# CVMI-Lab/HybridNeuralRendering

Measured on NVIDIA B200. Metric: train rays/s (fwd+bwd), higher is better.
Workload: dtype f32

## Files before the change

### hybridneuralrendering_b200/csrc/aggregate.cu

```cuda
#include "common.cuh"

#include "hnr.h"
#include "img_common.cuh"

namespace {

constexpr int F_EMB = 32;
constexpr int NF_FEAT = 3;
constexpr int NF_DIST = 5;
constexpr int NF_VIEW = 4;
constexpr int X0_W = F_EMB + 2 * NF_FEAT * F_EMB + 2 * NF_DIST * 6;
constexpr int E_W = 7;
constexpr int HID = 256;
constexpr int X5_W = HID + 2 * NF_VIEW * 3;
constexpr int AUX_C = 45;

__device__ __forceinline__ void rot3(const float* m, float x, float y, float z, float& ox, float& oy, float& oz) {
    ox = x * m[0] + y * m[3] + z * m[6];
    oy = x * m[1] + y * m[4] + z * m[7];
    oz = x * m[2] + y * m[5] + z * m[8];
}

__device__ __forceinline__ bool slot_masked(const int32_t* pidx, const uint8_t* mask, int64_t i) {
    return mask ? (mask[i] == 0) : (pidx[i] < 0);
}

__global__ void nbr_weights_kernel(const float* __restrict__ xyz, const float* __restrict__ conf, const int32_t* __restrict__ pidx,
                                   const uint8_t* __restrict__ mask, const float* __restrict__ loc_w, int64_t S, int K,
                                   float* __restrict__ weight, float* __restrict__ confc, uint8_t* __restrict__ valid) {
    int64_t s = (int64_t)blockIdx.x * blockDim.x + threadIdx.x;
    if (s >= S) return;
    const float lx = loc_w[s * 3], ly = loc_w[s * 3 + 1], lz = loc_w[s * 3 + 2];
    float sum = 0.f;
    bool any = false;
    for (int k = 0; k < K; ++k) {
        int64_t i = s * K + k;
        bool m = slot_masked(pidx, mask, i);
        int64_t g = max(pidx[i], 0);
        float dx = xyz[g * 3] - lx, dy = xyz[g * 3 + 1] - ly, dz = xyz[g * 3 + 2] - lz;
        float u = m ? 0.f : 1.f / fmaxf(sqrtf(dx * dx + dy * dy + dz * dz), 1e-6f);
        weight[i] = u;
        sum += u;
        any |= !m;
        if (confc) confc[i] = conf ? fminf(fmaxf(conf[g], 1e-4f), 1.f) : 1.f;
    }
    float inv = 1.f / fmaxf(sum, 1e-8f);
    for (int k = 0; k < K; ++k) weight[s * K + k] *= inv;
    if (valid) valid[s] = any ? 1 : 0;
}

__global__ void __launch_bounds__(256)
nbr_features_kernel(const float* __restrict__ xyz, const float* __restrict__ xyz_pers, const float* __restrict__ emb,
                    const float* __restrict__ color, const float* __restrict__ dir, const int32_t* __restrict__ pidx,
                    const int32_t* __restrict__ vlist, const float* __restrict__ loc_w, const float* __restrict__ loc_pers,
                    const float* __restrict__ raydirs, const float* __restrict__ cam, int64_t rows, int K, float* __restrict__ X0,
                    float* __restrict__ E) {
    const int lane = threadIdx.x & 31;
    const int64_t row = ((int64_t)blockIdx.x * blockDim.x + threadIdx.x) >> 5;
    if (row >= rows) return;
    const int64_t v = row / K;
    const int k = (int)(row - v * K);
    const int64_t s = vlist[v];
    const int64_t g = max(pidx[s * K + k], 0);
    float* x0 = X0 + row * X0_W;
    {
        float e = emb[g * F_EMB + lane];
        x0[lane] = e;
        float* pe = x0 + F_EMB + lane * (2 * NF_FEAT);
#pragma unroll
        for (int f = 0; f < NF_FEAT; ++f) {
            float sn, cs;
            sincosf(e * (float)(1 << f), &sn, &cs);
            pe[2 * f] = sn;
            pe[2 * f + 1] = cs;
        }
    }
    const float px = xyz[g * 3], py = xyz[g * 3 + 1], pz = xyz[g * 3 + 2];
    float d[6];
    {
        float wx = px - loc_w[s * 3], wy = py - loc_w[s * 3 + 1], wz = pz - loc_w[s * 3 + 2];
        rot3((cam + 12), wx, wy, wz, d[0], d[1], d[2]);
        float qx, qy, qz;
        if (xyz_pers) {
            qx = xyz_pers[g * 3]; qy = xyz_pers[g * 3 + 1]; qz = xyz_pers[g * 3 + 2];
        } else {
            float cx, cy, cz;
            rot3((cam + 3), px - cam[0], py - cam[1], pz - cam[2], cx, cy, cz);
            qx = cx / cz; qy = cy / cz; qz = cz;
        }
        const float sx = loc_pers[s * 3], sy = loc_pers[s * 3 + 1], sz = loc_pers[s * 3 + 2];
        d[3] = qx * qz - sx * sz;
        d[4] = qy * qz - sy * sz;
        d[5] = qz - sz;
    }
    if (lane < 6 * NF_DIST) {
        int c = lane / NF_DIST, f = lane - c * NF_DIST;
        float dv = d[0];
#pragma unroll
        for (int i = 1; i < 6; ++i) dv = (c == i) ? d[i] : dv;
        float sn, cs;
        sincosf(dv * (float)(1 << f), &sn, &cs);
        float* o = x0 + F_EMB + 2 * NF_FEAT * F_EMB + lane * 2;
        o[0] = sn;
        o[1] = cs;
    }
    if (lane < E_W) {
        float vx, vy, vz, rx, ry, rz;
        rot3((cam + 12), raydirs[s * 3], raydirs[s * 3 + 1], raydirs[s * 3 + 2], vx, vy, vz);
        rot3((cam + 12), dir[g * 3], dir[g * 3 + 1], dir[g * 3 + 2], rx, ry, rz);
        float out;
        if (lane < 3) out = color[g * 3 + lane];
        else if (lane == 3) out = rx - vx;
        else if (lane == 4) out = ry - vy;
        else if (lane == 5) out = rz - vz;
        else out = rx * vx + ry * vy + rz * vz;
        E[row * E_W + lane] = out;
    }
}

__global__ void __launch_bounds__(256)
nbr_features_bwd_kernel(const float* __restrict__ dX0, const float* __restrict__ dE, const float* __restrict__ emb,
                        const int32_t* __restrict__ pidx, const uint8_t* __restrict__ mask, const int32_t* __restrict__ vlist,
                        const float* __restrict__ raydirs, const float* __restrict__ cam, int64_t rows, int K, float* __restrict__ d_emb,
                        float* __restrict__ d_color, float* __restrict__ d_dir, int ldx) {
    const int lane = threadIdx.x & 31;
    const int64_t row = ((int64_t)blockIdx.x * blockDim.x + threadIdx.x) >> 5;
    if (row >= rows) return;
    const int64_t v = row / K;
    const int k = (int)(row - v * K);
    const int64_t s = vlist[v];
    if (slot_masked(pidx, mask, s * K + k)) return;
    const int64_t g = pidx[s * K + k];
    const float* dx = dX0 + row * ldx;
    if (d_emb) {
        float e = emb[g * F_EMB + lane];
        float acc = dx[lane];
        const float* dpe = dx + F_EMB + lane * (2 * NF_FEAT);
#pragma unroll
        for (int f = 0; f < NF_FEAT; ++f) {
            float fr = (float)(1 << f), sn, cs;
            sincosf(e * fr, &sn, &cs);
            acc += fr * (cs * dpe[2 * f] - sn * dpe[2 * f + 1]);
        }
        atomicAdd(&d_emb[g * F_EMB + lane], acc);
    }
    if (lane < 3) {
        const float* de = dE + row * E_W;
        if (d_color) atomicAdd(&d_color[g * 3 + lane], de[lane]);
        if (d_dir) {
            float vx, vy, vz;
            rot3((cam + 12), raydirs[s * 3], raydirs[s * 3 + 1], raydirs[s * 3 + 2], vx, vy, vz);
            float gx = de[3] + de[6] * vx, gy = de[4] + de[6] * vy, gz = de[5] + de[6] * vz;
            float o = gx * (cam + 12)[lane * 3] + gy * (cam + 12)[lane * 3 + 1] + gz * (cam + 12)[lane * 3 + 2];
            atomicAdd(&d_dir[g * 3 + lane], o);
        }
    }
}

__device__ __forceinline__ float softplus_t(float x) { return x > 20.f ? x : log1pf(expf(x)); }

__global__ void __launch_bounds__(256)
alpha_ksum_fwd_kernel(const float* __restrict__ H, const float* __restrict__ weight, const float* __restrict__ confc,
                      const int32_t* __restrict__ vlist, const float* __restrict__ w_alpha, const float* __restrict__ b_alpha,
                      const float* __restrict__ raydirs, const float* __restrict__ cam, int64_t Nv, int K, float* __restrict__ sigma,
                      float* __restrict__ X5, float* __restrict__ alpha_raw) {
    const int lane = threadIdx.x & 31;
    const int64_t v = ((int64_t)blockIdx.x * blockDim.x + threadIdx.x) >> 5;
    if (v >= Nv) return;
    const int64_t s = vlist[v];
    const float4* wa4 = reinterpret_cast<const float4*>(w_alpha) + lane * 2;
    const float4 wa0 = wa4[0], wa1 = wa4[1];
    float4 a0 = make_float4(0, 0, 0, 0), a1 = a0;
    float sg = 0.f;
    for (int k = 0; k < K; ++k) {
        const float4* h4 = reinterpret_cast<const float4*>(H + (v * K + k) * HID) + lane * 2;
        float4 h0 = h4[0], h1 = h4[1];
        float dot = h0.x * wa0.x + h0.y * wa0.y + h0.z * wa0.z + h0.w * wa0.w + h1.x * wa1.x + h1.y * wa1.y + h1.z * wa1.z + h1.w * wa1.w;
        float raw = warp_sum(dot) + b_alpha[0];
        float wc = weight[s * K + k] * (confc ? confc[s * K + k] : 1.f);
        sg += wc * softplus_t(raw - 1.f);
        a0.x += wc * h0.x; a0.y += wc * h0.y; a0.z += wc * h0.z; a0.w += wc * h0.w;
        a1.x += wc * h1.x; a1.y += wc * h1.y; a1.z += wc * h1.z; a1.w += wc * h1.w;
        if (lane == 0 && alpha_raw) alpha_raw[v * K + k] = raw;
    }
    float4* o4 = reinterpret_cast<float4*>(X5 + v * X5_W) + lane * 2;
    o4[0] = a0; o4[1] = a1;
    if (lane == 0) sigma[v] = sg;
    if (lane < 3 * NF_VIEW) {
        float vx, vy, vz;
        rot3((cam + 12), raydirs[s * 3], raydirs[s * 3 + 1], raydirs[s * 3 + 2], vx, vy, vz);
        int c = lane / NF_VIEW, f = lane - c * NF_VIEW;
        float val = c == 0 ? vx : (c == 1 ? vy : vz);
        float sn, cs;
        sincosf(val * (float)(1 << f), &sn, &cs);
        X5[v * X5_W + HID + lane] = sn;
        X5[v * X5_W + HID + 3 * NF_VIEW + lane] = cs;
    }
}

template <int KT>
__global__ void __launch_bounds__(256)
alpha_ksum_bwd_kernel(const float* __restrict__ H, const float* __restrict__ weight, const float* __restrict__ confc,
                      const int32_t* __restrict__ vlist, const float* __restrict__ w_alpha, const float* __restrict__ alpha_raw,
                      const float* __restrict__ d_sigma, const float* __restrict__ dX5, int64_t Nv, int K, float* __restrict__ dH,
                      float* __restrict__ d_wc, float* __restrict__ d_walpha, float* __restrict__ d_balpha) {
    const int lane = threadIdx.x & 31;
    const int64_t warp0 = ((int64_t)blockIdx.x * blockDim.x + threadIdx.x) >> 5;
    const int64_t nwarps = ((int64_t)gridDim.x * blockDim.x) >> 5;
    const float4* wa4 = reinterpret_cast<const float4*>(w_alpha) + lane * 2;
    const float4 wa0 = wa4[0], wa1 = wa4[1];
    float4 gw0 = make_float4(0, 0, 0, 0), gw1 = gw0;
    float gb = 0.f;
    for (int64_t v = warp0; v < Nv; v += nwarps) {
        const int64_t s = vlist[v];
        const float ds = d_sigma[v];
        const float4* g4 = reinterpret_cast<const float4*>(dX5 + v * X5_W) + lane * 2;
        const float4 g0 = g4[0], g1 = g4[1];
        const int KK = KT > 0 ? KT : K;
#pragma unroll
        for (int k = 0; k < KK; ++k) {
            const int64_t row = v * KK + k;
            const float4* h4 = reinterpret_cast<const float4*>(H + row * HID) + lane * 2;
            float4 h0 = h4[0], h1 = h4[1];
            float wc = weight[s * KK + k] * (confc ? confc[s * KK + k] : 1.f);
            float raw = alpha_raw[row] - 1.f;
            float sp = softplus_t(raw);
            float sgm = 1.f / (1.f + expf(-raw));
            float draw = wc * ds * sgm;
            float hd = h0.x * g0.x + h0.y * g0.y + h0.z * g0.z + h0.w * g0.w + h1.x * g1.x + h1.y * g1.y + h1.z * g1.z + h1.w * g1.w;
            hd = warp_sum(hd);
            if (lane == 0) d_wc[row] = sp * ds + hd;
            float4 o0, o1;
            o0.x = wc * g0.x + draw * wa0.x; o0.y = wc * g0.y + draw * wa0.y; o0.z = wc * g0.z + draw * wa0.z; o0.w = wc * g0.w + draw * wa0.w;
            o1.x = wc * g1.x + draw * wa1.x; o1.y = wc * g1.y + draw * wa1.y; o1.z = wc * g1.z + draw * wa1.z; o1.w = wc * g1.w + draw * wa1.w;
            float4* d4 = reinterpret_cast<float4*>(dH + row * HID) + lane * 2;
            d4[0] = o0; d4[1] = o1;
            gw0.x += draw * h0.x; gw0.y += draw * h0.y; gw0.z += draw * h0.z; gw0.w += draw * h0.w;
            gw1.x += draw * h1.x; gw1.y += draw * h1.y; gw1.z += draw * h1.z; gw1.w += draw * h1.w;
            gb += draw;
        }
    }
    __shared__ float red[8][HID + 1];
    {
        float* o = &red[threadIdx.x >> 5][lane * 8];
        o[0] = gw0.x; o[1] = gw0.y; o[2] = gw0.z; o[3] = gw0.w; o[4] = gw1.x; o[5] = gw1.y; o[6] = gw1.z; o[7] = gw1.w;
        if (lane == 0) red[threadIdx.x >> 5][HID] = gb;
    }
    __syncthreads();
    const int nw = blockDim.x >> 5;
    for (int c = threadIdx.x; c <= HID; c += blockDim.x) {
        float t = 0.f;
        for (int w = 0; w < nw; ++w) t += red[w][c];
        atomicAdd(c < HID ? d_walpha + c : d_balpha, t);
    }
}

__global__ void __launch_bounds__(256)
alpha_ksum_bwd_img_kernel(const uint8_t* __restrict__ himg, const float* __restrict__ weight, const float* __restrict__ confc,
                          const int32_t* __restrict__ vlist, const float* __restrict__ w_alpha, const float* __restrict__ alpha_raw,
                          const float* __restrict__ d_sigma, const float* __restrict__ dX5, int64_t Nv, uint8_t* __restrict__ dzimg,
                          float* __restrict__ d_wc, float* __restrict__ d_walpha, float* __restrict__ d_balpha, float* __restrict__ d_confc) {
    constexpr int KK = 8;
    const int lane = threadIdx.x & 31;
    const int64_t warp0 = ((int64_t)blockIdx.x * blockDim.x + threadIdx.x) >> 5;
    const int64_t nwarps = ((int64_t)gridDim.x * blockDim.x) >> 5;
    const float4* wa4 = reinterpret_cast<const float4*>(w_alpha) + lane * 2;
    const float4 wa0 = wa4[0], wa1 = wa4[1];
    const float wa[8] = {wa0.x, wa0.y, wa0.z, wa0.w, wa1.x, wa1.y, wa1.z, wa1.w};
    float gw[8];
#pragma unroll
    for (int i = 0; i < 8; ++i) gw[i] = 0.f;
    float gb = 0.f;
    for (int64_t v = warp0; v < Nv; v += nwarps) {
        const int64_t s = vlist[v];
        const float ds = d_sigma[v];
        const float4* g4 = reinterpret_cast<const float4*>(dX5 + v * X5_W) + lane * 2;
        const float4 g0 = g4[0], g1 = g4[1];
        const float g[8] = {g0.x, g0.y, g0.z, g0.w, g1.x, g1.y, g1.z, g1.w};
        uint4 hh[KK], hl[KK];
#pragma unroll
        for (int k = 0; k < KK; ++k) {
            const uint8_t* p = himg + img::piece_off(v * KK + k, lane, HID);
            hh[k] = __ldg(reinterpret_cast<const uint4*>(p));
            hl[k] = __ldg(reinterpret_cast<const uint4*>(p + img::plane_bytes(HID)));
        }
#pragma unroll
        for (int k = 0; k < KK; ++k) {
            const int64_t row = v * KK + k;
            float h[8];
            img::join8_bf16(hh[k], hl[k], h);
            const float wc = weight[s * KK + k] * (confc ? confc[s * KK + k] : 1.f);
            const float raw = alpha_raw[row] - 1.f;
            const float sp = softplus_t(raw);
            const float sgm = 1.f / (1.f + expf(-raw));
            const float draw = wc * ds * sgm;
            float hd = 0.f;
#pragma unroll
            for (int i = 0; i < 8; ++i) hd = fmaf(h[i], g[i], hd);
            hd = warp_sum(hd);
            if (lane == 0) {
                d_wc[row] = sp * ds + hd;
                if (d_confc) d_confc[s * KK + k] = (sp * ds + hd) * weight[s * KK + k];
            }
            float o[8];
#pragma unroll
            for (int i = 0; i < 8; ++i) {
                o[i] = (wc * g[i] + draw * wa[i]) * (h[i] > 0.f ? 1.f : 0.01f);
                gw[i] = fmaf(draw, h[i], gw[i]);
            }
            gb += draw;
            uint4 hi, lo;
            img::split8_bf16(o, hi, lo);
            uint8_t* q = dzimg + img::piece_off(row, lane, HID);
            *reinterpret_cast<uint4*>(q) = hi;
            *reinterpret_cast<uint4*>(q + img::plane_bytes(HID)) = lo;
        }
    }
    __shared__ float red[8][HID + 1];
    {
        float* o = &red[threadIdx.x >> 5][lane * 8];
#pragma unroll
        for (int i = 0; i < 8; ++i) o[i] = gw[i];
        if (lane == 0) red[threadIdx.x >> 5][HID] = gb;
    }
    __syncthreads();
    const int nw = blockDim.x >> 5;
    for (int c = threadIdx.x; c <= HID; c += blockDim.x) {
        float t = 0.f;
        for (int w = 0; w < nw; ++w) t += red[w][c];
        atomicAdd(c < HID ? d_walpha + c : d_balpha, t);
    }
}

__global__ void conf_bwd_kernel(const float* __restrict__ d_wc, const float* __restrict__ weight, const int32_t* __restrict__ vlist,
                                const int32_t* __restrict__ pidx, int64_t Nv, int K, float* __restrict__ d_conf) {
    int64_t i = (int64_t)blockIdx.x * blockDim.x + threadIdx.x;
    if (i >= Nv * K) return;
    int64_t v = i / K;
    int k = (int)(i - v * K);
    int64_t s = vlist[v];
    float w = weight[s * K + k];
    if (w == 0.f) return;
    atomicAdd(&d_conf[max(pidx[s * K + k], 0)], d_wc[i] * w);
}
__global__ void __launch_bounds__(256) conf_up_bwd_kernel(const float* __restrict__ d_confc, const int32_t* __restrict__ pidx, int64_t n,
                                                          float* __restrict__ d_conf) {
    double gm = 0.0;
    for (int64_t i = (int64_t)blockIdx.x * blockDim.x + threadIdx.x; i < n; i += (int64_t)gridDim.x * blockDim.x) {
        const float g = d_confc[i];
        const int p = pidx[i];
        if (p < 0) gm += (double)g;
        else if (g != 0.f) atomicAdd(&d_conf[p], g);
    }
#pragma unroll
    for (int o = 16; o > 0; o >>= 1) gm += __shfl_xor_sync(0xffffffffu, gm, o);
    __shared__ double red[8];
    if ((threadIdx.x & 31) == 0) red[threadIdx.x >> 5] = gm;
    __syncthreads();
    if (threadIdx.x == 0) {
        double t = 0.0;
        for (int w = 0; w < 8; ++w) t += red[w];
        if (t != 0.0) atomicAdd(&d_conf[0], (float)t);
    }
}

__global__ void project_views_kernel(const float* __restrict__ loc_w, const float* __restrict__ w2c, const float* __restrict__ Kmat,
                                     const float* __restrict__ campos, const float* __restrict__ campos_n, int V, int64_t S,
                                     float* __restrict__ xy, float* __restrict__ delta) {
    int64_t i = (int64_t)blockIdx.x * blockDim.x + threadIdx.x;
    if (i >= (int64_t)V * S) return;
    int v = (int)(i / S);
    int64_t s = i - (int64_t)v * S;
    const float x = loc_w[s * 3], y = loc_w[s * 3 + 1], z = loc_w[s * 3 + 2];
    const float* m = w2c + v * 16;
    float cx = x * m[0] + y * m[1] + z * m[2] + m[3];
    float cy = x * m[4] + y * m[5] + z * m[6] + m[7];
    float cz = x * m[8] + y * m[9] + z * m[10] + m[11];
    float ix = cx * Kmat[0] + cy * Kmat[1] + cz * Kmat[2];
    float iy = cx * Kmat[3] + cy * Kmat[4] + cz * Kmat[5];
    float iz = cx * Kmat[6] + cy * Kmat[7] + cz * Kmat[8];
    float den = iz + 1e-10f;
    xy[i * 2] = ix / den;
    xy[i * 2 + 1] = iy / den;
    if (delta) {
        float ax = x - campos[0], ay = y - campos[1], az = z - campos[2];
        float an = sqrtf(ax * ax + ay * ay + az * az) + 1e-6f;
        float bx = x - campos_n[v * 3], by = y - campos_n[v * 3 + 1], bz = z - campos_n[v * 3 + 2];
        float bn = sqrtf(bx * bx + by * by + bz * bz) + 1e-6f;
        delta[i * 3] = bx / bn - ax / an;
        delta[i * 3 + 1] = by / bn - ay / an;
        delta[i * 3 + 2] = bz / bn - az / an;
    }
}

struct hnr_pyramid_t {
    const float* lvl[4];
    float* grad[4];
    int h[4], w[4], c[4];
};

__device__ __forceinline__ void bilin_setup(int dst, int in_size, int out_size, int& i0, int& i1, float& l0, float& l1) {
    float scale = (float)in_size / (float)out_size;
    float src = scale * ((float)dst + 0.5f) - 0.5f;
    if (src < 0.f) src = 0.f;
    i0 = (int)src;
    if (i0 > in_size - 1) i0 = in_size - 1;
    i1 = i0 + ((i0 < in_size - 1) ? 1 : 0);
    l1 = src - (float)i0;
    l0 = 1.f - l1;
}

template <bool BWD>
__global__ void __launch_bounds__(256)
image_gather_kernel(hnr_pyramid_t P, const float* __restrict__ xy, const int32_t* __restrict__ vlist, int V, int64_t S, int64_t Nv,
                    float* __restrict__ aux, float* __restrict__ ok, const float* __restrict__ d_aux, int d_ld = AUX_C) {
    const int lane = threadIdx.x & 31;
    const int64_t wid = ((int64_t)blockIdx.x * blockDim.x + threadIdx.x) >> 5;
    if (wid >= (int64_t)V * Nv) return;
    const int v = (int)(wid / Nv);
    const int64_t n = wid - (int64_t)v * Nv;
    const int64_t s = vlist[n];
    const float fx = xy[((int64_t)v * S + s) * 2], fy = xy[((int64_t)v * S + s) * 2 + 1];
    int px = (int)fx, py = (int)fy;
    const int H = P.h[0], W = P.w[0];
    const bool inb = !(px < 0 || px >= W || py < 0 || py >= H);
    if (!BWD && lane == 0) ok[wid] = inb ? 1.f : 0.f;
    const bool zero = !inb || (px == 0 && py == 0);
    for (int ch = lane; ch < AUX_C; ch += 32) {
        int l = ch < 3 ? 0 : (ch < 9 ? 1 : (ch < 21 ? 2 : 3));
        int c = ch - (l == 0 ? 0 : (l == 1 ? 3 : (l == 2 ? 9 : 21)));
        if (!BWD) {
            float val = 0.f;
            if (!zero) {
                if (l == 0) {
                    val = P.lvl[0][(((int64_t)v * H + py) * W + px) * 3 + c];
                } else {
                    int y0, y1, x0, x1; float ly0, ly1, lx0, lx1;
                    bilin_setup(py, P.h[l], H, y0, y1, ly0, ly1);
                    bilin_setup(px, P.w[l], W, x0, x1, lx0, lx1);
                    const float* b = P.lvl[l] + (int64_t)v * P.h[l] * P.w[l] * P.c[l];
                    const int C = P.c[l], wl = P.w[l];
                    float v00 = b[((int64_t)y0 * wl + x0) * C + c], v01 = b[((int64_t)y0 * wl + x1) * C + c];
                    float v10 = b[((int64_t)y1 * wl + x0) * C + c], v11 = b[((int64_t)y1 * wl + x1) * C + c];
                    val = ly0 * (lx0 * v00 + lx1 * v01) + ly1 * (lx0 * v10 + lx1 * v11);
                }
            }
            aux[wid * AUX_C + ch] = val;
        } else {
            if (zero || l == 0) continue;
            float g = d_aux[wid * d_ld + ch];
            if (g == 0.f) continue;
            int y0, y1, x0, x1; float ly0, ly1, lx0, lx1;
            bilin_setup(py, P.h[l], H, y0, y1, ly0, ly1);
            bilin_setup(px, P.w[l], W, x0, x1, lx0, lx1);
            float* b = P.grad[l] + (int64_t)v * P.h[l] * P.w[l] * P.c[l];
            const int C = P.c[l], wl = P.w[l];
            atomicAdd(&b[((int64_t)y0 * wl + x0) * C + c], g * ly0 * lx0);
            atomicAdd(&b[((int64_t)y0 * wl + x1) * C + c], g * ly0 * lx1);
            atomicAdd(&b[((int64_t)y1 * wl + x0) * C + c], g * ly1 * lx0);
            atomicAdd(&b[((int64_t)y1 * wl + x1) * C + c], g * ly1 * lx1);
        }
    }
}

__global__ void __launch_bounds__(256)
image_gather_fwd_v2_kernel(hnr_pyramid_t P, const float* __restrict__ xy, const int32_t* __restrict__ vlist, int V, int64_t S, int64_t Nv,
                           float* __restrict__ aux, float* __restrict__ ok, int aux_ld, const float* __restrict__ delta) {
    const int q = threadIdx.x & 15;
    const int64_t pair = ((int64_t)blockIdx.x * blockDim.x + threadIdx.x) >> 4;
    if (pair >= (int64_t)V * Nv || q > 12) return;
    const int v = (int)(pair / Nv);
    const int64_t n = pair - (int64_t)v * Nv;
    const int64_t s = vlist[n];
    const float2 f = *reinterpret_cast<const float2*>(xy + ((int64_t)v * S + s) * 2);
    const int px = (int)f.x, py = (int)f.y;
    const int H = P.h[0], W = P.w[0];
    const bool inb = !(px < 0 || px >= W || py < 0 || py >= H);
    const bool zero = !inb || (px == 0 && py == 0);
    float* o = aux + pair * aux_ld;
    if (q == 12) {
        ok[pair] = inb ? 1.f : 0.f;
        if (delta) {
            const float* dp = delta + ((int64_t)v * S + s) * 3;
            o[AUX_C] = dp[0]; o[AUX_C + 1] = dp[1]; o[AUX_C + 2] = dp[2];
        }
        float r = 0.f, g = 0.f, b = 0.f;
        if (!zero) {
            const float* p0 = P.lvl[0] + (((int64_t)v * H + py) * W + px) * 3;
            r = p0[0]; g = p0[1]; b = p0[2];
        }
        o[0] = r; o[1] = g; o[2] = b;
        return;
    }
    const int l = q < 6 ? 3 : (q < 9 ? 2 : 1);
    const int grp = q < 6 ? q : (q < 9 ? q - 6 : q - 9);
    const int ch0 = l == 3 ? 21 + 4 * grp : (l == 2 ? 9 + 4 * grp : 3 + 2 * grp);
    float r0 = 0.f, r1 = 0.f, r2 = 0.f, r3 = 0.f;
    if (!zero) {
        int y0, y1, x0, x1; float ly0, ly1, lx0, lx1;
        const int hl = l == 3 ? P.h[3] : (l == 2 ? P.h[2] : P.h[1]), wl = l == 3 ? P.w[3] : (l == 2 ? P.w[2] : P.w[1]);
        const int C = l == 3 ? 24 : (l == 2 ? 12 : 6);
        const float* lv = l == 3 ? P.lvl[3] : (l == 2 ? P.lvl[2] : P.lvl[1]);
        bilin_setup(py, hl, H, y0, y1, ly0, ly1);
        bilin_setup(px, wl, W, x0, x1, lx0, lx1);
        const float* b = lv + (int64_t)v * hl * wl * C;
        const int o00 = (y0 * wl + x0) * C, o01 = (y0 * wl + x1) * C, o10 = (y1 * wl + x0) * C, o11 = (y1 * wl + x1) * C;
        if (l == 1) {
            const float2 a = *reinterpret_cast<const float2*>(b + o00 + 2 * grp), bq = *reinterpret_cast<const float2*>(b + o01 + 2 * grp);
            const float2 c = *reinterpret_cast<const float2*>(b + o10 + 2 * grp), d = *reinterpret_cast<const float2*>(b + o11 + 2 * grp);
            r0 = ly0 * (lx0 * a.x + lx1 * bq.x) + ly1 * (lx0 * c.x + lx1 * d.x);
            r1 = ly0 * (lx0 * a.y + lx1 * bq.y) + ly1 * (lx0 * c.y + lx1 * d.y);
        } else {
            const float4 a = *reinterpret_cast<const float4*>(b + o00 + 4 * grp), bq = *reinterpret_cast<const float4*>(b + o01 + 4 * grp);
            const float4 c = *reinterpret_cast<const float4*>(b + o10 + 4 * grp), d = *reinterpret_cast<const float4*>(b + o11 + 4 * grp);
            r0 = ly0 * (lx0 * a.x + lx1 * bq.x) + ly1 * (lx0 * c.x + lx1 * d.x);
            r1 = ly0 * (lx0 * a.y + lx1 * bq.y) + ly1 * (lx0 * c.y + lx1 * d.y);
            r2 = ly0 * (lx0 * a.z + lx1 * bq.z) + ly1 * (lx0 * c.z + lx1 * d.z);
            r3 = ly0 * (lx0 * a.w + lx1 * bq.w) + ly1 * (lx0 * c.w + lx1 * d.w);
        }
    }
    o[ch0] = r0; o[ch0 + 1] = r1;
    if (l != 1) { o[ch0 + 2] = r2; o[ch0 + 3] = r3; }
}

__device__ __forceinline__ void red_add_v4(float* p, float a, float b, float c, float d) {
    asm volatile("red.global.add.v4.f32 [%0], {%1, %2, %3, %4};" ::"l"(p), "f"(a), "f"(b), "f"(c), "f"(d) : "memory");
}
__device__ __forceinline__ void red_add_v2(float* p, float a, float b) {
    asm volatile("red.global.add.v2.f32 [%0], {%1, %2};" ::"l"(p), "f"(a), "f"(b) : "memory");
}
__global__ void __launch_bounds__(256)
image_gather_bwd_v2_kernel(hnr_pyramid_t P, const float* __restrict__ xy, const int32_t* __restrict__ vlist, int V, int64_t S, int64_t Nv,
                           const float* __restrict__ d_aux, int d_ld) {
    const int q = threadIdx.x & 15;
    const int64_t pair = ((int64_t)blockIdx.x * blockDim.x + threadIdx.x) >> 4;
    if (pair >= (int64_t)V * Nv || q > 11) return;
    const int v = (int)(pair / Nv);
    const int64_t n = pair - (int64_t)v * Nv;
    const int64_t s = vlist[n];
    const float2 f = *reinterpret_cast<const float2*>(xy + ((int64_t)v * S + s) * 2);
    const int px = (int)f.x, py = (int)f.y;
    const int H = P.h[0], W = P.w[0];
    const bool inb = !(px < 0 || px >= W || py < 0 || py >= H);
    if (!inb || (px == 0 && py == 0)) return;
    const int l = q < 6 ? 3 : (q < 9 ? 2 : 1);
    const int grp = q < 6 ? q : (q < 9 ? q - 6 : q - 9);
    const int ch0 = l == 3 ? 21 + 4 * grp : (l == 2 ? 9 + 4 * grp : 3 + 2 * grp);
    const float* gp = d_aux + pair * d_ld + ch0;
    const float g0 = gp[0], g1 = gp[1], g2 = l != 1 ? gp[2] : 0.f, g3 = l != 1 ? gp[3] : 0.f;
    if (g0 == 0.f && g1 == 0.f && g2 == 0.f && g3 == 0.f) return;
    int y0, y1, x0, x1; float ly0, ly1, lx0, lx1;
    const int hl = l == 3 ? P.h[3] : (l == 2 ? P.h[2] : P.h[1]), wl = l == 3 ? P.w[3] : (l == 2 ? P.w[2] : P.w[1]);
    const int C = l == 3 ? 24 : (l == 2 ? 12 : 6);
    float* lv = l == 3 ? P.grad[3] : (l == 2 ? P.grad[2] : P.grad[1]);
    bilin_setup(py, hl, H, y0, y1, ly0, ly1);
    bilin_setup(px, wl, W, x0, x1, lx0, lx1);
    float* b = lv + (int64_t)v * hl * wl * C + (l == 1 ? 2 * grp : 4 * grp);
    const int o00 = (y0 * wl + x0) * C, o01 = (y0 * wl + x1) * C, o10 = (y1 * wl + x0) * C, o11 = (y1 * wl + x1) * C;
    const float w00 = ly0 * lx0, w01 = ly0 * lx1, w10 = ly1 * lx0, w11 = ly1 * lx1;
    if (l == 1) {
        red_add_v2(b + o00, g0 * w00, g1 * w00); red_add_v2(b + o01, g0 * w01, g1 * w01);
        red_add_v2(b + o10, g0 * w10, g1 * w10); red_add_v2(b + o11, g0 * w11, g1 * w11);
    } else {
        red_add_v4(b + o00, g0 * w00, g1 * w00, g2 * w00, g3 * w00); red_add_v4(b + o01, g0 * w01, g1 * w01, g2 * w01, g3 * w01);
        red_add_v4(b + o10, g0 * w10, g1 * w10, g2 * w10, g3 * w10); red_add_v4(b + o11, g0 * w11, g1 * w11, g2 * w11, g3 * w11);
    }
}

__global__ void blend_fwd_kernel(const float* __restrict__ aux, const float* __restrict__ sig, const float* __restrict__ ok,
                                 const uint8_t* __restrict__ keep, int V, int64_t Nv, int aux_ld, float* __restrict__ merged, int merged_ld) {
    int64_t i = (int64_t)blockIdx.x * blockDim.x + threadIdx.x;
    if (i >= Nv * merged_ld) return;
    int64_t n = i / merged_ld;
    int c = (int)(i - n * merged_ld);
    if (c >= AUX_C) { merged[i] = 0.f; return; }
    float num = 0.f, den = 0.f;
    for (int v = 0; v < V; ++v) {
        float w = sig[(int64_t)v * Nv + n] * ok[(int64_t)v * Nv + n];
        num += aux[((int64_t)v * Nv + n) * aux_ld + c] * w;
        den += w;
    }
    float m = num / (den + 1e-6f);
    if (keep && !keep[n]) m = 0.f;
    merged[i] = m;
}

__global__ void __launch_bounds__(256)
blend_bwd_kernel(const float* __restrict__ aux, const float* __restrict__ sig, const float* __restrict__ ok,
                 const uint8_t* __restrict__ keep, const float* __restrict__ d_merged, int V, int64_t Nv, float* __restrict__ d_aux,
                 float* __restrict__ d_sig, int ald, int dld) {
    const int lane = threadIdx.x & 31;
    const int64_t n = ((int64_t)blockIdx.x * blockDim.x + threadIdx.x) >> 5;
    if (n >= Nv) return;
    const bool kept = !(keep && !keep[n]);
    float den = 1e-6f;
    for (int v = 0; v < V; ++v) den += sig[(int64_t)v * Nv + n] * ok[(int64_t)v * Nv + n];
    float dm[2], mr[2];
    for (int j = 0; j < 2; ++j) {
        int c = lane + 32 * j;
        dm[j] = (c < AUX_C && kept) ? d_merged[n * AUX_C + c] : 0.f;
        float num = 0.f;
        if (c < AUX_C)
            for (int v = 0; v < V; ++v) num += aux[((int64_t)v * Nv + n) * ald + c] * sig[(int64_t)v * Nv + n] * ok[(int64_t)v * Nv + n];
        mr[j] = num / den;
    }
    for (int v = 0; v < V; ++v) {
        const int64_t r = (int64_t)v * Nv + n;
// ... 211 lines not shown
```

### hybridneuralrendering_b200/csrc/nbr_bwd_f16.cu

```cuda
#include "common.cuh"
#include "hnr.h"
#define TRACE_SRC ((long long*)nullptr)
#include "tc_common.cuh"
#include "img_common.cuh"

namespace {
using namespace tc;

constexpr int TM = 128;
constexpr int HID = 256;
constexpr int KC = 16;
constexpr int NSW = 3, NSA = 3, NSG = 3;
constexpr int W_PART = HID * KC * 2;
constexpr int W_STAGE = 2 * W_PART;
constexpr int A_PART = TM * KC * 2;
constexpr int A_STAGE = 2 * A_PART;
constexpr int G_STAGE = TM * 32 * 2;
constexpr int ACT_PART = TM * HID * 2;
constexpr int NLAYER = 4, NC = HID / KC;
constexpr int NITEM = NC + 3 * 8;
constexpr int DEPTH = 4;
constexpr int NEPI = 256, NTHREADS = 512;
static_assert(NITEM % DEPTH == 0, "the loader's register queue must line up across tiles");

constexpr int OFF_W = 0;
constexpr int OFF_A = OFF_W + NSW * W_STAGE;
constexpr int OFF_G = OFF_A + NSA * A_STAGE;
constexpr int OFF_ACT = OFF_G + NSG * G_STAGE;
constexpr int OFF_BAR = OFF_ACT + 2 * ACT_PART;
constexpr int NBAR = 2 * NSW + 2 * NSA + 2 * NSG + 8 + 2 + 2;
constexpr int SMEM_BYTES = OFF_BAR + NBAR * 8 + 16;
static_assert(SMEM_BYTES <= 227 * 1024, "shared memory budget");

constexpr uint32_t IDESC = (1u << 4) | (1u << 7) | (1u << 10) | ((uint32_t)(HID >> 3) << 17) | ((uint32_t)(TM >> 4) << 24);
constexpr uint32_t A_LBO = (TM / 8) * 128, W_LBO = (HID / 8) * 128, SBO = 128;
constexpr int64_t IMG_SLAB = 256 * 128, IMG_PLANE = 256 * 64;

struct BArgs {
    const uint8_t* dz3;
    const uint8_t* h[3];
    uint8_t* dz[3];
    float* dX0;
    const uint8_t* wpack;
    int64_t rows;
    int ldx, nx0;
};

__device__ __forceinline__ void tc_mma_bf16(uint32_t d_tmem, uint64_t a_desc, uint64_t b_desc, uint32_t idesc, uint32_t accumulate) {
    asm volatile(
        "{\n\t.reg .pred p;\n\t"
        "setp.ne.b32 p, %4, 0;\n\t"
        "tcgen05.mma.cta_group::1.kind::f16 [%0], %1, %2, %3, p;\n\t}"
        ::"r"(d_tmem), "l"(a_desc), "l"(b_desc), "r"(idesc), "r"(accumulate)
        : "memory");
}
__device__ __forceinline__ void tmem_ld32_issue(uint32_t taddr, uint32_t (&r)[32]) {
    asm volatile(
        "tcgen05.ld.sync.aligned.32x32b.x32.b32 "
        "{%0, %1, %2, %3, %4, %5, %6, %7, %8, %9, %10, %11, %12, %13, %14, %15, "
        "%16, %17, %18, %19, %20, %21, %22, %23, %24, %25, %26, %27, %28, %29, %30, %31}, [%32];"
        : "=r"(r[0]), "=r"(r[1]), "=r"(r[2]), "=r"(r[3]), "=r"(r[4]), "=r"(r[5]), "=r"(r[6]), "=r"(r[7]), "=r"(r[8]), "=r"(r[9]),
          "=r"(r[10]), "=r"(r[11]), "=r"(r[12]), "=r"(r[13]), "=r"(r[14]), "=r"(r[15]), "=r"(r[16]), "=r"(r[17]), "=r"(r[18]),
          "=r"(r[19]), "=r"(r[20]), "=r"(r[21]), "=r"(r[22]), "=r"(r[23]), "=r"(r[24]), "=r"(r[25]), "=r"(r[26]), "=r"(r[27]),
          "=r"(r[28]), "=r"(r[29]), "=r"(r[30]), "=r"(r[31])
        : "r"(taddr)
        : "memory");
}
__device__ __forceinline__ void tmem_ld_wait(uint32_t (&r)[32]) {
    asm volatile("tcgen05.wait::ld.sync.aligned;"
                 : "+r"(r[0]), "+r"(r[1]), "+r"(r[2]), "+r"(r[3]), "+r"(r[4]), "+r"(r[5]), "+r"(r[6]), "+r"(r[7]), "+r"(r[8]), "+r"(r[9]),
                   "+r"(r[10]), "+r"(r[11]), "+r"(r[12]), "+r"(r[13]), "+r"(r[14]), "+r"(r[15]), "+r"(r[16]), "+r"(r[17]), "+r"(r[18]),
                   "+r"(r[19]), "+r"(r[20]), "+r"(r[21]), "+r"(r[22]), "+r"(r[23]), "+r"(r[24]), "+r"(r[25]), "+r"(r[26]), "+r"(r[27]),
                   "+r"(r[28]), "+r"(r[29]), "+r"(r[30]), "+r"(r[31])
                 :
                 : "memory");
}
__device__ __forceinline__ void mbar_wait_relaxed(uint32_t bar, uint32_t parity, unsigned ns) {
    uint32_t done;
    for (;;) {
        asm volatile(
            "{\n\t.reg .pred p;\n\t"
            "mbarrier.try_wait.parity.shared::cta.b64 p, [%1], %2;\n\t"
            "selp.u32 %0, 1, 0, p;\n\t}"
            : "=r"(done)
            : "r"(bar), "r"(parity)
            : "memory");
        if (done) break;
        __nanosleep(ns);
    }
}
template <int N>
__device__ __forceinline__ void setmaxnreg_inc() { asm volatile("setmaxnreg.inc.sync.aligned.u32 %0;" ::"n"(N)); }
template <int N>
__device__ __forceinline__ void setmaxnreg_dec() { asm volatile("setmaxnreg.dec.sync.aligned.u32 %0;" ::"n"(N)); }

__device__ __forceinline__ uint4 ldg16(const uint8_t* p) { return __ldg(reinterpret_cast<const uint4*>(p)); }

__device__ __forceinline__ float slope_lo(uint32_t p) { return img::bf16_lo_f(p) > 0.f ? 1.f : 0.01f; }
__device__ __forceinline__ float slope_hi(uint32_t p) { return img::bf16_hi_f(p) > 0.f ? 1.f : 0.01f; }

__global__ void __launch_bounds__(NTHREADS, 1) nbr_bwd_f16_kernel(const __grid_constant__ BArgs A) {
    extern __shared__ __align__(1024) uint8_t smem[];
    const int tid = threadIdx.x, warp = tid >> 5, lane = tid & 31;
    uint64_t* bars = reinterpret_cast<uint64_t*>(smem + OFF_BAR);
    const uint32_t b0 = smem_u32(bars);
    const uint32_t bar_wfull = b0, bar_wempty = bar_wfull + 8 * NSW, bar_afull = bar_wempty + 8 * NSW, bar_aempty = bar_afull + 8 * NSA,
                   bar_gfull = bar_aempty + 8 * NSA, bar_gempty = bar_gfull + 8 * NSG, bar_actfull = bar_gempty + 8 * NSG,
                   bar_accfull = bar_actfull + 64, bar_accempty = bar_accfull + 16;
    uint32_t* tmem_slot = reinterpret_cast<uint32_t*>(bars + NBAR);
    const int64_t ntiles = (A.rows + TM - 1) / TM;

    if (tid == 0) {
        for (int s = 0; s < NSW; ++s) { mbar_init(bar_wfull + 8 * s, 1); mbar_init(bar_wempty + 8 * s, 1); }
        for (int s = 0; s < NSA; ++s) { mbar_init(bar_afull + 8 * s, 4); mbar_init(bar_aempty + 8 * s, 1); }
        for (int s = 0; s < NSG; ++s) { mbar_init(bar_gfull + 8 * s, 4); mbar_init(bar_gempty + 8 * s, 4); }
        for (int s = 0; s < 8; ++s) mbar_init(bar_actfull + 8 * s, 4);
        for (int s = 0; s < 2; ++s) { mbar_init(bar_accfull + 8 * s, 1); mbar_init(bar_accempty + 8 * s, 8); }
        asm volatile("fence.mbarrier_init.release.cluster;" ::: "memory");
    }
    if (warp == 12) tmem_alloc(smem_u32(tmem_slot), 512);
    tc_fence_before();
    __syncthreads();
    tc_fence_after();
    const uint32_t tmem_base = *tmem_slot;

    if (warp >= 12) {
        setmaxnreg_dec<40>();
        if (warp == 13 && lane == 0) {
            uint32_t it = 0;
            for (int64_t tile = blockIdx.x; tile < ntiles; tile += gridDim.x) {
                for (int c = 0; c < NLAYER * NC; ++c, ++it) {
                    const uint32_t s = it % NSW, ph = (it / NSW) & 1;
                    mbar_wait_relaxed(bar_wempty + 8 * s, ph ^ 1, 64);
                    mbar_arrive_expect_tx(bar_wfull + 8 * s, W_STAGE);
                    bulk_g2s(smem_u32(smem + OFF_W + s * W_STAGE), A.wpack + (size_t)c * W_STAGE, W_STAGE, bar_wfull + 8 * s);
                }
            }
        } else if (warp == 12) {
            uint32_t wit = 0, ait = 0, gen = 0, ti = 0;
            const uint32_t act_hi = smem_u32(smem + OFF_ACT), act_lo = act_hi + ACT_PART;
            const uint32_t w_base = smem_u32(smem + OFF_W), a_base = smem_u32(smem + OFF_A);
            const uint64_t dW = umma_desc(0, W_LBO, SBO), dA = umma_desc(0, A_LBO, SBO);
            auto issue = [&](uint32_t acc, uint32_t a_hi_addr, uint32_t a_lo_addr, bool first, uint32_t extra_commit) {
                const uint32_t s = wit % NSW, ph = (wit / NSW) & 1;
                ++wit;
                mbar_wait(bar_wfull + 8 * s, ph);
                tc_fence_after();
                if (elect_one()) {
                    const uint32_t w = w_base + s * W_STAGE;
                    const uint64_t w_hi = dW | (uint64_t)((w & 0x3FFFFu) >> 4), w_lo = dW | (uint64_t)(((w + W_PART) & 0x3FFFFu) >> 4);
                    const uint64_t a_hi = dA | (uint64_t)((a_hi_addr & 0x3FFFFu) >> 4), a_lo = dA | (uint64_t)((a_lo_addr & 0x3FFFFu) >> 4);
                    tc_mma_bf16(acc, a_hi, w_hi, IDESC, first ? 0u : 1u);
                    tc_mma_bf16(acc, a_lo, w_hi, IDESC, 1u);
                    tc_mma_bf16(acc, a_hi, w_lo, IDESC, 1u);
                    tc_commit(bar_wempty + 8 * s);
                    if (extra_commit) tc_commit(extra_commit);
                }
                __syncwarp();
            };
            for (int64_t tile = blockIdx.x; tile < ntiles; tile += gridDim.x, ++ti) {
                const uint32_t acc0 = tmem_base, acc1 = tmem_base + HID;
                if (ti > 0) mbar_wait(bar_accempty, (ti - 1) & 1);
                for (int c = 0; c < NC; ++c, ++ait) {
                    const uint32_t s = ait % NSA, ph = (ait / NSA) & 1;
                    mbar_wait_relaxed(bar_afull + 8 * s, ph, 20);
                    const uint32_t a = a_base + s * A_STAGE;
                    issue(acc0, a, a + A_PART, c == 0, bar_aempty + 8 * s);
                }
                if (elect_one()) tc_commit(bar_accfull);
                __syncwarp();
                if (ti > 0) mbar_wait(bar_accempty + 8, (ti - 1) & 1);
#pragma unroll 1
                for (int j = 1; j < NLAYER; ++j) {
                    const uint32_t acc = (j & 1) ? acc1 : acc0;
                    for (int c = 0; c < NC; ++c) {
                        if ((c & 1) == 0) mbar_wait_relaxed(bar_actfull + 8 * (c >> 1), gen & 1, 20);
                        issue(acc, act_hi + c * 2 * A_LBO, act_lo + c * 2 * A_LBO, c == 0, 0);
                    }
                    if (elect_one()) tc_commit(bar_accfull + 8 * (j & 1));
                    __syncwarp();
                    ++gen;
                }
            }
        }
    } else if (warp >= 8) {
        setmaxnreg_dec<120>();
        const int r = tid - NEPI;
        uint32_t ait = 0, git = 0;
        uint4 q[DEPTH][4];
        auto load_item = [&](int64_t tile, int i, uint4 (&d)[4]) {
            if (tile >= ntiles) return;
            const int64_t row = tile * TM + r;
            const int64_t ro = (row >> 5) * IMG_SLAB + (row & 31) * 16;
            if (i < NC) {
                if (row < A.rows) {
                    const uint8_t* p = A.dz3 + ro + (int64_t)(2 * i) * 512;
                    d[0] = ldg16(p); d[1] = ldg16(p + 512); d[2] = ldg16(p + IMG_PLANE); d[3] = ldg16(p + IMG_PLANE + 512);
                } else {
                    d[0] = d[1] = d[2] = d[3] = make_uint4(0u, 0u, 0u, 0u);
                    uint8_t* p = const_cast<uint8_t*>(A.dz3) + ro + (int64_t)(2 * i) * 512;
                    *reinterpret_cast<uint4*>(p) = d[0]; *reinterpret_cast<uint4*>(p + 512) = d[0];
                    *reinterpret_cast<uint4*>(p + IMG_PLANE) = d[0]; *reinterpret_cast<uint4*>(p + IMG_PLANE + 512) = d[0];
                }
            } else {
                const int j = (i - NC) >> 3, jb = (i - NC) & 7;
                const uint8_t* p = (j == 0 ? A.h[0] : (j == 1 ? A.h[1] : A.h[2])) + ro + (int64_t)(4 * jb) * 512;
                d[0] = ldg16(p); d[1] = ldg16(p + 512); d[2] = ldg16(p + 1024); d[3] = ldg16(p + 1536);
            }
        };
        auto put_item = [&](int i, const uint4 (&d)[4]) {
            if (i < NC) {
                const uint32_t st = ait % NSA, ph = (ait / NSA) & 1;
                ++ait;
                mbar_wait_relaxed(bar_aempty + 8 * st, ph ^ 1, 32);
                uint8_t* stage = smem + OFF_A + st * A_STAGE + r * 16;
                *reinterpret_cast<uint4*>(stage) = d[0];
                *reinterpret_cast<uint4*>(stage + A_LBO) = d[1];
                *reinterpret_cast<uint4*>(stage + A_PART) = d[2];
                *reinterpret_cast<uint4*>(stage + A_PART + A_LBO) = d[3];
                fence_proxy_async();
                __syncwarp();
                if (lane == 0) mbar_arrive(bar_afull + 8 * st);
            } else {
                const uint32_t st = git % NSG, ph = (git / NSG) & 1;
                ++git;
                mbar_wait_relaxed(bar_gempty + 8 * st, ph ^ 1, 32);
                uint8_t* stage = smem + OFF_G + st * G_STAGE + r * 16;
#pragma unroll
                for (int k = 0; k < 4; ++k) *reinterpret_cast<uint4*>(stage + k * 2048) = d[k];
                __syncwarp();
                if (lane == 0) mbar_arrive(bar_gfull + 8 * st);
            }
        };
#pragma unroll
        for (int i = 0; i < DEPTH; ++i) load_item(blockIdx.x, i, q[i]);
        for (int64_t tile = blockIdx.x; tile < ntiles; tile += gridDim.x) {
#pragma unroll
            for (int i = 0; i < NITEM; ++i) {
                put_item(i, q[i % DEPTH]);
                if (i + DEPTH < NITEM) load_item(tile, i + DEPTH, q[i % DEPTH]);
                else load_item(tile + gridDim.x, i + DEPTH - NITEM, q[i % DEPTH]);
            }
        }
    } else {
        setmaxnreg_inc<168>();
        const int wg = warp >> 2;
        const int r = tid & (TM - 1);
        const uint32_t lane_base = (uint32_t)(32 * (warp & 3)) << 16;
        uint8_t* act_hi = smem + OFF_ACT;
        uint32_t ti = 0;
        for (int64_t tile = blockIdx.x; tile < ntiles; tile += gridDim.x, ++ti) {
            const int64_t row = tile * TM + r;
            const int64_t ro = (row >> 5) * IMG_SLAB + (row & 31) * 16;
#pragma unroll 1
            for (int j = 0; j < NLAYER; ++j) {
                const uint32_t b = j & 1;
                mbar_wait_relaxed(bar_accfull + 8 * b, (j >> 1) & 1, 20);
                tc_fence_after();
                const uint32_t taddr = tmem_base + lane_base + b * HID + wg * 32;
                uint32_t va[32], vb[32];
                tmem_ld32_issue(taddr, va);
                if (j < NLAYER - 1) {
                    uint8_t* out = j == 0 ? A.dz[0] : (j == 1 ? A.dz[1] : A.dz[2]);
#pragma unroll
                    for (int jj = 0; jj < 4; ++jj) {
                        const int jb = 2 * jj + wg;
                        uint32_t(&cur)[32] = (jj & 1) ? vb : va;
                        uint32_t(&nxt)[32] = (jj & 1) ? va : vb;
                        const uint32_t gi = ti * 24u + (uint32_t)j * 8u + (uint32_t)jb, st = gi % NSG, ph = (gi / NSG) & 1;
                        mbar_wait_relaxed(bar_gfull + 8 * st, ph, 20);
                        uint4 g4[4];
#pragma unroll
                        for (int k = 0; k < 4; ++k) g4[k] = *reinterpret_cast<const uint4*>(smem + OFF_G + st * G_STAGE + k * 2048 + r * 16);
                        __syncwarp();
                        if (lane == 0) mbar_arrive(bar_gempty + 8 * st);
                        tmem_ld_wait(cur);
                        if (jj + 1 < 4) tmem_ld32_issue(taddr + (jj + 1) * 64, nxt);
#pragma unroll
                        for (int qd = 0; qd < 4; ++qd) {
                            const uint32_t gw[4] = {g4[qd].x, g4[qd].y, g4[qd].z, g4[qd].w};
                            float y[8];
#pragma unroll
                            for (int u = 0; u < 4; ++u) {
                                y[2 * u] = __uint_as_float(cur[8 * qd + 2 * u]) * slope_lo(gw[u]);
                                y[2 * u + 1] = __uint_as_float(cur[8 * qd + 2 * u + 1]) * slope_hi(gw[u]);
                            }
                            uint4 hi, lo;
                            img::split8_bf16(y, hi, lo);
                            uint8_t* dst = act_hi + (jb * 4 + qd) * A_LBO + r * 16;
                            *reinterpret_cast<uint4*>(dst) = hi;
                            *reinterpret_cast<uint4*>(dst + ACT_PART) = lo;
                            uint8_t* gdst = out + ro + (int64_t)(jb * 4 + qd) * 512;
                            *reinterpret_cast<uint4*>(gdst) = hi;
                            *reinterpret_cast<uint4*>(gdst + IMG_PLANE) = lo;
                        }
                        fence_proxy_async();
                        __syncwarp();
                        if (lane == 0) mbar_arrive(bar_actfull + 8 * jb);
                    }
                    if (j == 2) {
                        tc_fence_before();
                        __syncwarp();
                        if (lane == 0) mbar_arrive(bar_accempty);
                    }
                } else {
#pragma unroll
                    for (int jj = 0; jj < 4; ++jj) {
                        const int jb = 2 * jj + wg;
                        uint32_t(&cur)[32] = (jj & 1) ? vb : va;
                        uint32_t(&nxt)[32] = (jj & 1) ? va : vb;
                        tmem_ld_wait(cur);
                        if (jj + 1 < 4) tmem_ld32_issue(taddr + (jj + 1) * 64, nxt);
                        if (row < A.rows && jb * 32 < A.nx0) {
                            float4* o = reinterpret_cast<float4*>(A.dX0 + row * A.ldx + jb * 32);
#pragma unroll
                            for (int i = 0; i < 8; ++i)
                                o[i] = make_float4(__uint_as_float(cur[4 * i]), __uint_as_float(cur[4 * i + 1]), __uint_as_float(cur[4 * i + 2]),
                                                   __uint_as_float(cur[4 * i + 3]));
                        }
                    }
                    tc_fence_before();
                    __syncwarp();
                    if (lane == 0) mbar_arrive(bar_accempty + 8);
                }
            }
        }
    }
    tc_fence_before();
    __syncthreads();
    if (warp == 12) tmem_dealloc(tmem_base, 512);
}

__global__ void __launch_bounds__(128) dz_extras_kernel(const uint8_t* __restrict__ dz, const float* __restrict__ W, int ldw, int k0,
                                                        int64_t rows, float* __restrict__ dE) {
    __shared__ float ws[HID * 8];
    for (int i = threadIdx.x; i < HID * 8; i += blockDim.x) {
        const int n = i >> 3, jx = i & 7;
        ws[i] = jx < 7 ? W[(int64_t)n * ldw + k0 + jx] : 0.f;
    }
    __syncthreads();
    const int64_t row = (int64_t)blockIdx.x * blockDim.x + threadIdx.x;
    if (row >= rows) return;
    const uint8_t* p = dz + (row >> 5) * IMG_SLAB + (row & 31) * 16;
    float acc[7];
#pragma unroll
    for (int jx = 0; jx < 7; ++jx) acc[jx] = 0.f;
#pragma unroll 4
    for (int g = 0; g < HID / 8; ++g) {
        const uint4 hi = ldg16(p + g * 512), lo = ldg16(p + IMG_PLANE + g * 512);
        float v[8];
        img::join8_bf16(hi, lo, v);
#pragma unroll
        for (int u = 0; u < 8; ++u) {
            const float4 w0 = *reinterpret_cast<const float4*>(ws + (g * 8 + u) * 8), w1 = *reinterpret_cast<const float4*>(ws + (g * 8 + u) * 8 + 4);
            acc[0] = fmaf(v[u], w0.x, acc[0]); acc[1] = fmaf(v[u], w0.y, acc[1]); acc[2] = fmaf(v[u], w0.z, acc[2]); acc[3] = fmaf(v[u], w0.w, acc[3]);
            acc[4] = fmaf(v[u], w1.x, acc[4]); acc[5] = fmaf(v[u], w1.y, acc[5]); acc[6] = fmaf(v[u], w1.z, acc[6]);
        }
    }
#pragma unroll
    for (int jx = 0; jx < 7; ++jx) dE[row * 7 + jx] = acc[jx];
}

}

extern "C" int64_t hnr_nbr_bwd_f16_packed_bytes(void) { return (int64_t)NLAYER * NC * W_STAGE; }

extern "C" int hnr_nbr_bwd_f16(const void* dz3, const void* h2, const void* h1, const void* h0, void* dz2, void* dz1, void* dz0, float* dX0,
                               int64_t ldx, int64_t nx0, const void* wpackT, int64_t rows, void* stream) {
    if (rows == 0) return HNR_OK;
    HNR_CHECK_ARG(nx0 > 0 && nx0 % 32 == 0 && nx0 <= HID && ldx >= nx0 && ldx % 4 == 0, "nbr_bwd_f16: nx0 must be a multiple of 32 <= 256, ldx % 4 == 0");
    BArgs A{};
    A.dz3 = (const uint8_t*)dz3; A.h[0] = (const uint8_t*)h2; A.h[1] = (const uint8_t*)h1; A.h[2] = (const uint8_t*)h0;
    A.dz[0] = (uint8_t*)dz2; A.dz[1] = (uint8_t*)dz1; A.dz[2] = (uint8_t*)dz0; A.dX0 = dX0; A.ldx = (int)ldx; A.nx0 = (int)nx0;
    A.wpack = (const uint8_t*)wpackT; A.rows = rows;
    static bool configured = false;
    if (!configured) {
        HNR_CUDA(cudaFuncSetAttribute(nbr_bwd_f16_kernel, cudaFuncAttributeMaxDynamicSharedMemorySize, SMEM_BYTES));
        configured = true;
    }
    const int64_t ntiles = hnr_cdiv(rows, TM);
    const int grid = (int)(ntiles < HNR_NUM_SMS ? ntiles : HNR_NUM_SMS);
    nbr_bwd_f16_kernel<<<grid, NTHREADS, SMEM_BYTES, (cudaStream_t)stream>>>(A);
    HNR_CHECK_LAUNCH("nbr_bwd_f16");
    return HNR_OK;
}

extern "C" int hnr_dz_extras_bwd(const void* dz, const float* W, int64_t ldw, int64_t k0, int64_t rows, float* dE, void* stream) {
    if (rows == 0) return HNR_OK;
    dz_extras_kernel<<<(unsigned)hnr_cdiv(rows, 128), 128, 0, (cudaStream_t)stream>>>((const uint8_t*)dz, W, (int)ldw, (int)k0, rows, dE);
    HNR_CHECK_LAUNCH("dz_extras_bwd");
    return HNR_OK;
}
```

Before: 511,100.

## Batch alpha-bwd warp reductions and stage dX0 epilogue stores through shared memory

```diff
diff --git a/hybridneuralrendering_b200/csrc/aggregate.cu b/hybridneuralrendering_b200/csrc/aggregate.cu
--- a/hybridneuralrendering_b200/csrc/aggregate.cu
+++ b/hybridneuralrendering_b200/csrc/aggregate.cu
@@ -261,16 +261,20 @@
                           const float* __restrict__ d_sigma, const float* __restrict__ dX5, int64_t Nv, uint8_t* __restrict__ dzimg,
                           float* __restrict__ d_wc, float* __restrict__ d_walpha, float* __restrict__ d_balpha, float* __restrict__ d_confc) {
     constexpr int KK = 8;
+    constexpr unsigned FULL = 0xffffffffu;
     const int lane = threadIdx.x & 31;
     const int64_t warp0 = ((int64_t)blockIdx.x * blockDim.x + threadIdx.x) >> 5;
     const int64_t nwarps = ((int64_t)gridDim.x * blockDim.x) >> 5;
     const float4* wa4 = reinterpret_cast<const float4*>(w_alpha) + lane * 2;
     const float4 wa0 = wa4[0], wa1 = wa4[1];
     const float wa[8] = {wa0.x, wa0.y, wa0.z, wa0.w, wa1.x, wa1.y, wa1.z, wa1.w};
+    const bool up4 = lane & 16, up3 = lane & 8, up2 = lane & 4;
+    const int kr = lane & 7, kq = lane >> 2;
     float gw[8];
 #pragma unroll
     for (int i = 0; i < 8; ++i) gw[i] = 0.f;
     float gb = 0.f;
+#pragma unroll 1
     for (int64_t v = warp0; v < Nv; v += nwarps) {
         const int64_t s = vlist[v];
         const float ds = d_sigma[v];
@@ -284,25 +288,43 @@
             hh[k] = __ldg(reinterpret_cast<const uint4*>(p));
             hl[k] = __ldg(reinterpret_cast<const uint4*>(p + img::plane_bytes(HID)));
         }
+        const float w_r = weight[s * KK + kr];
+        const float wc_r = w_r * (confc ? confc[s * KK + kr] : 1.f);
+        const float raw = alpha_raw[v * KK + kr] - 1.f;
+        const float sp_r = softplus_t(raw);
+        const float sgm = 1.f / (1.f + expf(-raw));
+        const float draw_r = wc_r * ds * sgm;
+        float hd[KK];
+#pragma unroll
+        for (int k = 0; k < KK; ++k) {
+            float h[8];
+            img::join8_bf16(hh[k], hl[k], h);
+            hd[k] = 0.f;
+#pragma unroll
+            for (int i = 0; i < 8; ++i) hd[k] = fmaf(h[i], g[i], hd[k]);
+        }
+        float a4[4], a2[2];
+#pragma unroll
+        for (int i = 0; i < 4; ++i) a4[i] = (up4 ? hd[i + 4] : hd[i]) + __shfl_xor_sync(FULL, up4 ? hd[i] : hd[i + 4], 16);
+#pragma unroll
+        for (int i = 0; i < 2; ++i) a2[i] = (up3 ? a4[i + 2] : a4[i]) + __shfl_xor_sync(FULL, up3 ? a4[i] : a4[i + 2], 8);
+        float hd_q = (up2 ? a2[1] : a2[0]) + __shfl_xor_sync(FULL, up2 ? a2[0] : a2[1], 4);
+        hd_q += __shfl_xor_sync(FULL, hd_q, 2);
+        hd_q += __shfl_xor_sync(FULL, hd_q, 1);
+        {
+            const float sp = __shfl_sync(FULL, sp_r, kq), w = __shfl_sync(FULL, w_r, kq);
+            if ((lane & 3) == 0) {
+                const float dwc = sp * ds + hd_q;
+                d_wc[v * KK + kq] = dwc;
+                if (d_confc) d_confc[s * KK + kq] = dwc * w;
+            }
+        }
 #pragma unroll
         for (int k = 0; k < KK; ++k) {
             const int64_t row = v * KK + k;
-            float h[8];
+            const float wc = __shfl_sync(FULL, wc_r, k), draw = __shfl_sync(FULL, draw_r, k);
+            float h[8], o[8];
             img::join8_bf16(hh[k], hl[k], h);
-            const float wc = weight[s * KK + k] * (confc ? confc[s * KK + k] : 1.f);
-            const float raw = alpha_raw[row] - 1.f;
-            const float sp = softplus_t(raw);
-            const float sgm = 1.f / (1.f + expf(-raw));
-            const float draw = wc * ds * sgm;
-            float hd = 0.f;
-#pragma unroll
-            for (int i = 0; i < 8; ++i) hd = fmaf(h[i], g[i], hd);
-            hd = warp_sum(hd);
-            if (lane == 0) {
-                d_wc[row] = sp * ds + hd;
-                if (d_confc) d_confc[s * KK + k] = (sp * ds + hd) * weight[s * KK + k];
-            }
-            float o[8];
 #pragma unroll
             for (int i = 0; i < 8; ++i) {
                 o[i] = (wc * g[i] + draw * wa[i]) * (h[i] > 0.f ? 1.f : 0.01f);
diff --git a/hybridneuralrendering_b200/csrc/nbr_bwd_f16.cu b/hybridneuralrendering_b200/csrc/nbr_bwd_f16.cu
--- a/hybridneuralrendering_b200/csrc/nbr_bwd_f16.cu
+++ b/hybridneuralrendering_b200/csrc/nbr_bwd_f16.cu
@@ -244,9 +244,9 @@
         }
     } else {
         setmaxnreg_inc<168>();
-        const int wg = warp >> 2;
+        const int wg = warp >> 2, slab = warp & 3;
         const int r = tid & (TM - 1);
-        const uint32_t lane_base = (uint32_t)(32 * (warp & 3)) << 16;
+        const uint32_t lane_base = (uint32_t)(32 * slab) << 16;
         uint8_t* act_hi = smem + OFF_ACT;
         uint32_t ti = 0;
         for (int64_t tile = blockIdx.x; tile < ntiles; tile += gridDim.x, ++ti) {
@@ -304,6 +304,7 @@
                         if (lane == 0) mbar_arrive(bar_accempty);
                     }
                 } else {
+                    const int64_t row0 = tile * TM + 32 * slab;
 #pragma unroll
                     for (int jj = 0; jj < 4; ++jj) {
                         const int jb = 2 * jj + wg;
@@ -311,12 +312,26 @@
                         uint32_t(&nxt)[32] = (jj & 1) ? va : vb;
                         tmem_ld_wait(cur);
                         if (jj + 1 < 4) tmem_ld32_issue(taddr + (jj + 1) * 64, nxt);
-                        if (row < A.rows && jb * 32 < A.nx0) {
-                            float4* o = reinterpret_cast<float4*>(A.dX0 + row * A.ldx + jb * 32);
-#pragma unroll
-                            for (int i = 0; i < 8; ++i)
-                                o[i] = make_float4(__uint_as_float(cur[4 * i]), __uint_as_float(cur[4 * i + 1]), __uint_as_float(cur[4 * i + 2]),
-                                                   __uint_as_float(cur[4 * i + 3]));
+                        if (jb * 32 < A.nx0) {
+                            uint8_t* const stage = act_hi + jb * 4 * A_LBO + slab * 512;
+                            {
+                                const int k = lane >> 2;
+                                uint8_t* w = stage + (k & 1) * ACT_PART + (k >> 1) * A_LBO + (lane & 3) * 128;
+#pragma unroll
+                                for (int i = 0; i < 8; ++i)
+                                    *reinterpret_cast<uint4*>(w + ((i ^ (lane & 7)) << 4)) = make_uint4(cur[4 * i], cur[4 * i + 1], cur[4 * i + 2], cur[4 * i + 3]);
+                            }
+                            __syncwarp();
+                            const int c = lane & 7, q = lane >> 3;
+                            const uint8_t* rd = stage + q * 128;
+                            float* o = A.dX0 + (row0 + q) * A.ldx + jb * 32 + c * 4;
+                            const int64_t left = A.rows - (row0 + q);
+#pragma unroll
+                            for (int t = 0; t < 8; ++t) {
+                                const uint4 v = *reinterpret_cast<const uint4*>(rd + (t & 1) * ACT_PART + (t >> 1) * A_LBO + ((c ^ q ^ ((t & 1) << 2)) << 4));
+                                if (4 * t < left) *reinterpret_cast<uint4*>(o + (int64_t)(4 * t) * A.ldx) = v;
+                            }
+                            __syncwarp();
                         }
                     }
                     tc_fence_before();
```

Result: no change. 519,000, median of 6 (+1.5%).
